# dvrp0/Monsoon

Hardware: AMD Instinct MI355X
Metric: env-steps/sec (whole node) at 65536 concurrent games; bit-exact vs CPU replay (higher is better)
Workload: dtype u8/i16 state, f64 draw+score

## Files before the change

monsoon_amd/csrc/msb_base.h:

```cpp
#pragma once
#include <stdint.h>

#if defined(__HIPCC__)
#include <hip/hip_runtime.h>
#define MSB_HD __device__
#define MSB_NOINLINE __attribute__((noinline))
#else
#define MSB_HD
#define MSB_NOINLINE __attribute__((noinline))
#endif
#define MSB_INL inline __attribute__((always_inline))

#define MSB_PROF_LDS 16
#if defined(MSB_PROF) && MSB_PROF && defined(__HIP_DEVICE_COMPILE__)
typedef __attribute__((address_space(3))) unsigned long long* msb_lds64;
typedef __attribute__((address_space(3))) unsigned* msb_lds32;
__device__ inline __attribute__((always_inline)) bool msb_prof_leader() {
  unsigned l = __builtin_amdgcn_mbcnt_hi(~0u, __builtin_amdgcn_mbcnt_lo(~0u, 0u));
  return (unsigned)__builtin_amdgcn_readfirstlane((int)l) == l;
}
struct ProfScope {
  unsigned long long t0;
  int id;
  __device__ inline __attribute__((always_inline)) explicit ProfScope(int i) : t0(__builtin_readcyclecounter()), id(i) {
    if (msb_prof_leader()) {
      unsigned long long pre = *(msb_lds64)(unsigned long)(MSB_PROF_LDS + 896);
      if (pre) {
        __hip_atomic_fetch_add((msb_lds64)(unsigned long)(MSB_PROF_LDS + 384 + 8 * id), t0 - pre, __ATOMIC_RELAXED, __HIP_MEMORY_SCOPE_WORKGROUP);
        *(msb_lds64)(unsigned long)(MSB_PROF_LDS + 896) = 0ull;
      }
    }
  }
  __device__ inline __attribute__((always_inline)) ~ProfScope() {
    unsigned long long now = __builtin_readcyclecounter();
    if (msb_prof_leader()) {
      __hip_atomic_fetch_add((msb_lds64)(unsigned long)(MSB_PROF_LDS + 8 * id), now - t0, __ATOMIC_RELAXED, __HIP_MEMORY_SCOPE_WORKGROUP);
      __hip_atomic_fetch_add((msb_lds32)(unsigned long)(MSB_PROF_LDS + 256 + 4 * id), 1u, __ATOMIC_RELAXED, __HIP_MEMORY_SCOPE_WORKGROUP);
      *(msb_lds64)(unsigned long)(MSB_PROF_LDS + 904) = now;
    }
  }
};
#define MSB_SCOPE(id) ProfScope msb_prof_scope_(id)
#define MSB_PRECALL()                                                                                   \
  do {                                                                                                  \
    if (msb_prof_leader()) *(msb_lds64)(unsigned long)(MSB_PROF_LDS + 896) = __builtin_readcyclecounter(); \
  } while (0)
#define MSB_POSTCALL(id)                                                                                \
  do {                                                                                                  \
    unsigned long long now_ = __builtin_readcyclecounter();                                             \
    if (msb_prof_leader()) {                                                                            \
      unsigned long long post_ = *(msb_lds64)(unsigned long)(MSB_PROF_LDS + 904);                       \
      if (post_ && now_ > post_)                                                                        \
        __hip_atomic_fetch_add((msb_lds64)(unsigned long)(MSB_PROF_LDS + 640 + 8 * (id)), now_ - post_, __ATOMIC_RELAXED, __HIP_MEMORY_SCOPE_WORKGROUP); \
      *(msb_lds64)(unsigned long)(MSB_PROF_LDS + 904) = 0ull;                                           \
    }                                                                                                   \
  } while (0)
#else
#define MSB_SCOPE(id)
#define MSB_PRECALL() do {} while (0)
#define MSB_POSTCALL(id) do {} while (0)
#endif
enum {
  PS_STEP, PS_PLAYER_PLAY, PS_NEW_ENTITY, PS_RUN_ABILITY, PS_ABILITY_ENTITY, PS_ABILITY_SPELL, PS_GET_TARGETS, PS_SHAPE_TILES,
  PS_SHAPE_TARGETS, PS_DEAL_DAMAGE, PS_DESTROY, PS_FRONT_LINE, PS_SET_PATH, PS_MOVE, PS_COMMAND, PS_FORCE_ATTACK, PS_DRAW,
  PS_FLIP, PS_NEXT_TURN, PS_LEGAL, PS_SHUFFLE, PS_SORTED_HEAD, PS_SPAWN, PS_RESPAWN, PS_TELEPORT, PS_PUSH_PULL, PS_EMPTY_FRONT,
  PS_BEGIN_STEP, PS_OBS_RAISES, PS_FEATURES, PS_COUNT
};


namespace msb {

enum : int { KIND_UNIT = 0, KIND_STRUCT = 1, KIND_SPELL = 2 };
enum : int { TR_NONE = -1, TR_ON_PLAY = 0, TR_ON_DEATH = 1, TR_BEFORE_ATTACKING = 2, TR_AFTER_ATTACKING = 3,
             TR_AFTER_SURVIVING = 4, TR_BEFORE_MOVING = 5, TR_TURN_START = 6, TR_TURN_END = 7 };
enum : int { ST_FROZEN = 0, ST_POISONED = 1, ST_CONFUSED = 2, ST_DISABLED = 3, ST_VITALIZED = 4 };
enum : int { PH_TURN_START = 0, PH_PLAY = 1, PH_TURN_END = 2 };
enum : int { UT_CONSTRUCT = 0, UT_FLAKE, UT_KNIGHT, UT_PIRATE, UT_RAVEN, UT_RODENT, UT_SATYR, UT_TOAD, UT_UNDEAD,
             UT_VIKING, UT_HERO, UT_DRAGON, UT_ELDER, UT_FELINE, UT_ANCIENT, UT_PRIMAL };
enum : int { TK_UNIT = 0, TK_STRUCTURE = 1, TK_ANY = 2 };
enum : int { TS_FRIENDLY = 0, TS_ENEMY = 1, TS_ANY = 2 };

enum : int {
  FAULT_NONE = 0,
  FAULT_PY_EXCEPTION = 1,
  FAULT_INT_CARD = 2,
  FAULT_CAPACITY = 16,
  FAULT_TRIG_STACK = 17,
  FAULT_DEPTH = 18,
  FAULT_RNG_OVERRUN = 19,
  FAULT_UNSUPPORTED = 20,
  FAULT_STATUS_SAT = 21,
  FAULT_CAP_REM = 22,
  FAULT_CAP_DECK = 23,
  FAULT_CAP_HAND = 24,
  FAULT_CAP_PATH = 25,
  FAULT_CAP_INST = 26,
  FAULT_BOT_BOUND = 27,
  FAULT_OPP_BOUND = 28,
  FAULT_WORK_STACK = 29,
};

struct TargetSpec {
  int8_t has, kind, side;
  uint16_t types, xtypes;
  int16_t limit;
  int8_t non_hero;
  uint8_t status, xstatus;
  int8_t base;
};
struct CardInfo {
  int8_t kind, faction;
  uint8_t cost, strength, movement;
  int8_t trigger, ff, has_ability;
  uint16_t types;
  int8_t first_type;
  int32_t int_id;
  TargetSpec tgt;
};

// ... 42 lines not shown
```

monsoon_amd/csrc/rules.h:

```cpp
#pragma once
#include "mt19937.h"
#include "pyset.h"
#include "state.h"

#if defined(MSB_FAULT_TRACE) && !defined(__HIPCC__)
#include <execinfo.h>
#include <stdio.h>
static inline void msb_fault_trace(int code) {
  void* bt[24];
  int n = backtrace(bt, 24);
  fprintf(stderr, "set_fault(%d)\n", code);
  backtrace_symbols_fd(bt, n, 2);
}
#endif

#if defined(MSB_COUNT_FRAMES) && !defined(__HIPCC__)
#define MSB_COUNT_EVENT(i_) msb_frame_count[i_]++
#define MSB_COUNT_MAX(i_, v_) (msb_frame_count[i_] = (v_) > msb_frame_count[i_] ? (v_) : msb_frame_count[i_])
static long long msb_frame_count[64];
#else
#define MSB_COUNT_EVENT(i_)
#define MSB_COUNT_MAX(i_, v_)
#endif

// ... 296 lines not shown
    for (int i = j; i + 1 < n; i++) m.st8(pl(o, P_DECK + i), m.ld8(pl(o, P_DECK + i + 1)));
#else
    for (int i = j; i + 1 < n; i++) {
      m.st32(pl(o, P_DECK + 4 * i), m.ld32(pl(o, P_DECK + 4 * (i + 1))));
      m.st8(pl(o, P_AGE + i), m.ld8(pl(o, P_AGE + i + 1)));
    }
    m.st8(pl(o, P_AGE + n - 1), 0);
#endif
    m.st8(pl(o, P_DECK_N), n - 1);
  }
  MSB_HD MSB_INL void hand_remove_at(int o, int j) {
    int n = pl_hand_n(o);
#if defined(MSB_EXT) && MSB_EXT
    for (int i = j; i + 1 < n; i++) m.st8(pl(o, P_HAND + i), m.ld8(pl(o, P_HAND + i + 1)));
#else
    for (int i = j; i + 1 < n; i++) m.st32(pl(o, P_HAND + 4 * i), m.ld32(pl(o, P_HAND + 4 * (i + 1))));
#endif
    m.st8(pl(o, P_HAND_N), n - 1);
  }
  MSB_HD MSB_INL void hand_push_from_deck(int o, int idx) {
    int hn = pl_hand_n(o);
    if (hn >= HAND_CAP) {
      set_fault(FAULT_CAP_HAND);
      return;
    }
#if defined(MSB_EXT) && MSB_EXT
    m.st8(pl(o, P_HAND + hn), deck_id(o, idx));
#else
    m.st32(pl(o, P_HAND + 4 * hn), m.ld32(pl(o, P_DECK + 4 * idx)));
#endif
    m.st8(pl(o, P_HAND_N), hn + 1);
  }
  MSB_HD MSB_INL uint32_t hand_handle(int o, int i) const {
#if defined(MSB_EXT) && MSB_EXT
    return (uint32_t)hand_id(o, i);
#else
    return m.ld32(pl(o, P_HAND + 4 * i));
#endif
  }
  MSB_HD MSB_INL void deck_push_handle(int o, uint32_t h) {
    int n = pl_deck_n(o);
    if (n >= DECK_CAP) {
      set_fault(FAULT_CAP_DECK);
      return;
    }
#if defined(MSB_EXT) && MSB_EXT
    m.st8(pl(o, P_DECK + n), (int)h);
#else
    m.st32(pl(o, P_DECK + 4 * n), h);
    m.st8(pl(o, P_AGE + n), 0);
#endif
    m.st8(pl(o, P_DECK_N), n + 1);
  }
  MSB_HD MSB_NOINLINE void push_new_instance(int o, bool to_hand, int card, int cost, int fl, int x) {
    int n = to_hand ? pl_hand_n(o) : pl_deck_n(o);
    if (n >= (to_hand ? HAND_CAP : DECK_CAP)) {
      set_fault(to_hand ? FAULT_CAP_HAND : FAULT_CAP_DECK);
      return;
    }
    int rec, wrec = -1;
#if defined(MSB_EXT) && MSB_EXT
    int id = inst_alloc(o);
    if (fault()) return;
    m.st8(pl(o, (to_hand ? P_HAND : P_DECK) + n), id);
    rec = pl(o, P_INST + 4 * id);
    wrec = pl(o, P_AGE + id);
    m.st8(pl(o, P_IPOS + id), IPOS_UNKNOWN);
#else
    rec = pl(o, (to_hand ? P_HAND : P_DECK) + 4 * n);
    if (!to_hand) wrec = pl(o, P_AGE + n);
#endif
    m.st8(rec, card);
    m.st8(rec + 1, cost);
    m.st8(rec + 2, fl);
    m.st8(rec + 3, x);
    if (wrec >= 0) m.st8(wrec, 0);
    m.st8(pl(o, to_hand ? P_HAND_N : P_DECK_N), n + 1);
  }

  MSB_HD MSB_INL int board_at(int tile) const { return m.ld8(OFF_BOARD + tile); }
  MSB_HD MSB_INL void board_put(int tile, int slot) { m.st8(OFF_BOARD + tile, slot); }

  MSB_HD MSB_INL static int ent(int e) { return OFF_ENT + ENT_SIZE * e; }
  static_assert(OFF_ENT % 16 == 0 && ENT_SIZE == 16 && OFF_PL % 16 == 0 && PL_SIZE % 16 == 0, "granule-aligned blocks");
  MSB_HD MSB_INL static int eg(int e) { return OFF_ENT / 16 + e; }
  MSB_HD MSB_INL static int pg(int order) { return OFF_PL / 16 + order * (PL_SIZE / 16); }
  MSB_HD MSB_INL int e_card(int e) const { return m.ld8g(eg(e), EO_CARD); }
  MSB_HD MSB_INL int e_flags(int e) const { return m.ld8g(eg(e), EO_FLAGS); }
  MSB_HD MSB_INL int e_owner(int e) const { return m.ld8g(eg(e), EO_FLAGS) & EF_OWNER; }
  MSB_HD MSB_INL bool e_ff(int e) const { return (m.ld8g(eg(e), EO_FLAGS) & EF_FF) != 0; }
  MSB_HD MSB_INL void e_set_flag(int e, int bit, bool on) {
    int f = m.ld8g(eg(e), EO_FLAGS);
    m.st8g(eg(e), EO_FLAGS, on ? (f | bit) : (f & ~bit));
  }
  MSB_HD MSB_INL P e_pos(int e) const { return tile_p(m.ld8g(eg(e), EO_POS)); }
  MSB_HD MSB_INL void e_set_pos(int e, P p) { m.st8g(eg(e), EO_POS, p_tile(p)); }
  MSB_HD MSB_INL int e_mov(int e) const { return m.ld8g(eg(e), EO_MOV); }
  MSB_HD MSB_INL int e_str(int e) const { return m.ld16g(eg(e), EO_STR); }
  MSB_HD MSB_INL void e_set_str(int e, int v) { m.st16g(eg(e), EO_STR, v); }
  MSB_HD MSB_INL int e_dmg(int e) const { return m.ld16g(eg(e), EO_DMG); }
  MSB_HD MSB_INL void e_set_dmg(int e, int v) { m.st16g(eg(e), EO_DMG, v); }
  MSB_HD MSB_INL int e_st(int e, int s) const { return m.ld8g(eg(e), EO_ST + s); }
  MSB_HD MSB_INL void e_st_add(int e, int s) {
    int c = m.ld8g(eg(e), EO_ST + s);
    if (c >= 255) {
      set_fault(FAULT_STATUS_SAT);
// ... 1057 lines not shown
      if (e_card_trigger(e) == TR_ON_DEATH) {
        push_trigger(e, src);
        if (fault()) return;
        if (!m.ld8(H_RESOLVING)) {
          wk_push(k, mk_hdr(F_DESTROY_TAIL, 0, 0, 0));
          call_pop_trigger(k);
          return;
        }
      }
      recalc_front_after_destroy();
    } else {
      e_set_dmg(e, e_str(e));
      board_set(e_pos(e), -1);
      recalc_front_after_destroy();
    }
  }
  MSB_HD MSB_INL bool need_unit(int e) {
    if (e < 0 || e >= AT_PLAYER || !e_is_unit(e)) {
      set_fault(FAULT_PY_EXCEPTION);
      return false;
    }
    return true;
  }
  MSB_HD MSB_INL void freeze(int e) {
    if (need_unit(e)) e_st_add(e, ST_FROZEN);
  }
  MSB_HD MSB_INL void poison(int e) {
    if (!need_unit(e)) return;
    if (e_st(e, ST_VITALIZED) > 0) e_st_remove(e, ST_VITALIZED);
    e_st_add(e, ST_POISONED);
  }
  MSB_HD MSB_INL void vitalize(int e) {
    if (!need_unit(e)) return;
    if (e_st(e, ST_POISONED) > 0) e_st_remove(e, ST_POISONED);
    e_st_add(e, ST_VITALIZED);
  }
  MSB_HD MSB_INL void confuse(int e) {
    if (need_unit(e)) e_st_add(e, ST_CONFUSED);
  }
  MSB_HD MSB_INL void deconfuse(int e) {
    if (need_unit(e)) e_st_remove(e, ST_CONFUSED);
  }
  MSB_HD MSB_INL void disable(int e) {
    if (need_unit(e) && e_has_ability(e)) e_st_add(e, ST_DISABLED);
  }

  MSB_HD MSB_INL void set_path(int e, bool on_play) {
    const int sv = ctx_enter(e);
    set_path_impl(e, on_play);
    ctx_leave(sv);
  }
  MSB_HD MSB_A_SETPATH void set_path_impl(int e, bool on_play) {
    MSB_SCOPE(PS_SET_PATH);
    P position = e_pos(e);
    int confused_cached = e_st(e, ST_CONFUSED);
    int owner = e_owner(e);
    bool is_local = owner == local();
    int steps = on_play ? e_mov(e) : 1;
    uint32_t packed = 0;
    int n = 0;
    unsigned long long dests = 0;
    int nd = 0;
    for (int k = 0; k < steps; k++) {
      P dest{position.x, position.y + (is_local ? -1 : 1)};
      int nxt = at(dest);
      if (confused_cached > 0) {
        int dx;
        if (position.x == 0)
          dx = 1;
        else if (position.x == 3)
          dx = -1;
        else
          dx = rng_randint(0, 2) ? 1 : -1;
        dest = P{position.x + dx, position.y};
        confused_cached--;
      } else if (on_play && !e_ff(e) && dest.y != (is_local ? -1 : 5) &&
                 (nxt == AT_NONE || (nxt < AT_PLAYER && e_owner(nxt) == owner))) {
        P lp{position.x - 1, position.y}, rp{position.x + 1, position.y};
        int left = position.x > 0 ? at(lp) : AT_NONE;
        int right = position.x < 3 ? at(rp) : AT_NONE;
        bool left_ok = left >= 0 && left < AT_PLAYER && e_owner(left) != owner;
        bool right_ok = right >= 0 && right < AT_PLAYER && e_owner(right) != owner;
        int lpk = p_pack(lp), rpk = p_pack(rp);
        bool lseen = false, rseen = false;
        for (int i = 0; i < nd; i++) {
          int dv = (int)((dests >> (8 * i)) & 0xff);
          if (dv == lpk) lseen = true;
          if (dv == rpk) rseen = true;
        }
        if (position.x <= 1) {
          if (right_ok && !rseen)
            dest = rp;
          else if (left_ok && !lseen)
            dest = lp;
        } else {
          if (left_ok && !lseen)
            dest = lp;
          else if (right_ok && !rseen)
            dest = rp;
        }
      }
      P enc = dest;
      if (enc.y < -1) enc.y = -1;
      if (enc.y > 5) enc.y = 5;
      if (nd < 8) dests |= (unsigned long long)p_pack(enc) << (8 * nd++);
      if (n < PATH_CAP) {
        packed |= (uint32_t)p_pack(enc) << (8 * n);
        n++;
      } else {
        set_fault(FAULT_CAP_PATH);
      }
      position = dest;
    }
    e_set_path(e, packed);
    m.st8g(eg(e), EO_PATHN, n);
  }

  enum : int { MV_ENTRY = 0, MV_POISONED, MV_BEFORE_MOVING, MV_STEP, MV_BASE_HIT, MV_FIGHT, MV_STRUCK, MV_STRUCK_BACK,
               MV_TARGET_DEAD, MV_SELF_DEAD, MV_AFTER_ATTACK, MV_DONE, MV_START };
  static constexpr int MV_PLAYED = 0x80;
  MSB_HD MSB_INL int move_enter(Wk& k, int e) {
    const int sv = ctx_enter(e);
    if (fault()) return -1;
    wk_push_ctx(k, sv);
    const int d = m.ld8(H_DEPTH);
    if (d >= MAX_DEPTH || !wk_reserve(k)) {
      MSB_COUNT_MAX(12, k.base + k.sp - k.seg);
      set_fault(d >= MAX_DEPTH ? FAULT_DEPTH : FAULT_WORK_STACK);
      return -1;
    }
    m.st8(H_DEPTH, d + 1);
    MSB_COUNT_MAX(13, d + 1);
    return d;
  }
  MSB_HD MSB_INL void call_move(Wk& k, int e, int played = 0) {
    const int d = move_enter(k, e);
    if (d < 0) return;
    k.sp += 3;
    wk_push(k, mk_hdr(F_MOVE, MV_ENTRY, e, d | played));
  }
  MSB_HD MSB_INL void call_move_later(Wk& k, int e, int played) {
    k.sp += 3;
    wk_push(k, mk_hdr(F_MOVE, MV_START, e, played));
  }
  MSB_HD MSB_INL void h_move(Wk& k, uint32_t hdr) {
    if (hdr_st(hdr) == MV_START) {
      const int e0 = hdr_a(hdr), played = hdr_b(hdr) & MV_PLAYED;
      k.sp -= 4;
      const int d0 = move_enter(k, e0);
      if (d0 < 0) return;
      k.sp += 4;
      hdr = mk_hdr(F_MOVE, MV_ENTRY, e0, d0 | played);
    }
    const int top = k.sp - 1;
    const int e = hdr_a(hdr), d = hdr_b(hdr) & 0x7f;
    const int played_tail = hdr_b(hdr) & MV_PLAYED;
    uint32_t path = 0, w2 = 0;
    int cached = 0;
    if (hdr_st(hdr) != MV_ENTRY) {
      path = m.sk_ld(top - 1);
      w2 = m.sk_ld(top - 2);
      cached = (int)(int16_t)(m.sk_ld(top - 3) & 0xffffu);
    }
    int i = (int)(w2 & 7), n = (int)((w2 >> 3) & 7), current_id = (int)((w2 >> 8) & 0xff), target = (int)((w2 >> 16) & 0xff);
    int flags = (int)(w2 >> 24);
    const int trig = e_trigger(e);
    int next = MV_DONE;
    P dest{0, 0};
// ... 314 lines not shown
    return !(acc / last <= u);
  }
  MSB_HD MSB_A_DRAW void draw(int o, int amount, int hint = 0) {
    MSB_SCOPE(PS_DRAW);
    for (int k = 0; k < amount; k++) {
      int n = pl_deck_n(o);
      if (n == 0) {
        set_fault(FAULT_PY_EXCEPTION);
        return;
      }
      int idx = 0;
      if (k == 0 && hint > 0) {
        (void)rng_random_sample();
        idx = hint - 1;
      } else {
        double sum = 0.0;
        for (int i = 0; i < n; i++) sum = sum + deck_w(o, i);
        double last = 0.0;
        for (int i = 0; i < n; i++) {
          double p = deck_w(o, i) / sum;
          last = (i == 0) ? p : last + p;
        }
        double u = rng_random_sample();
        double acc = 0.0;
        for (; idx < n; idx++) {
          double p = deck_w(o, idx) / sum;
          acc = (idx == 0) ? p : acc + p;
          if (draw_stops(acc, last, u)) break;
        }
#if defined(MSB_STUDY_DRAW)
        {
          double sum2 = 0.0, last2 = 0.0, acc2 = 0.0;
          for (int i = 0; i < n; i++) sum2 = sum2 + deck_w(o, i);
          asm volatile("" : "+v"(sum2));
          for (int i = 0; i < n; i++) {
            double p = deck_w(o, i) / sum2;
            last2 = (i == 0) ? p : last2 + p;
          }
          asm volatile("" : "+v"(last2));
          int idx2 = 0;
          for (; idx2 < n; idx2++) {
            double p = deck_w(o, idx2) / sum2;
            acc2 = (idx2 == 0) ? p : acc2 + p;
            if (draw_stops(acc2, last2, u)) break;
          }
          asm volatile("" : : "v"(idx2), "v"(acc2) : "memory");
        }
#endif
      }
      if (idx >= n) {
        set_fault(FAULT_PY_EXCEPTION);
        return;
      }
      set_deck_age(o, idx, 0);
      hand_push_from_deck(o, idx);
      if (fault()) return;
      int j = first_equal(o, false, idx);
      if (fault()) return;
      deck_remove_at(o, j);
    }
  }
  MSB_HD MSB_INL void fill_hand(int o) {
    int need = 4 - pl_hand_n(o);
    if (need > 0) draw(o, need);
  }
  MSB_HD MSB_INL void discard(int o, int hand_index) {
    reweight(o);
    if (fault()) return;
    uint32_t target = hand_handle(o, hand_index);
    int fl = hand_flags(o, hand_index);
    int j = first_equal(o, true, hand_index);
    if (fault()) return;
    hand_remove_at(o, j);
    if (!(fl & CF_SINGLE_USE)) deck_push_handle(o, target);
  }
  MSB_HD MSB_INL void add_history(int owner, int card) {
    int n = m.ld8(H_HIST_N);
    uint64_t h = m.ld64(H_HIST);
    const uint64_t entry = (uint64_t)(owner & 0xff) | ((uint64_t)(card & 0xff) << 8);
    if (n < 4) {
      h = (h & ~(0xffffull << (16 * n))) | (entry << (16 * n));
      m.st8(H_HIST_N, n + 1);
    } else {
      h = (h >> 16) | (entry << 48);
    }
    m.st64(H_HIST, h);
  }
  MSB_HD MSB_INL void call_player_play(Wk& k, int o, int index, P position, bool has_pos) {
    MSB_SCOPE(PS_PLAYER_PLAY);
    int card = hand_card(o, index), fl = hand_flags(o, index);
    int strength = inst_strength(card, fl, hand_x(o, index));
    add_history(o, card);
    discard(o, index);
    if (fault()) return;
    const CardInfo& ci = g_cards[card];
    if (ci.kind == KIND_UNIT) {
      int e = new_entity(card, o, strength, ci.movement, (fl & CF_FF) != 0);
      if (fault()) return;
      if (!has_pos) {
        set_fault(FAULT_PY_EXCEPTION);
        return;
      }
      call_unit_play(k, e, position);
    } else if (ci.kind == KIND_STRUCT) {
      int e = new_entity(card, o, strength, 0, false);
      if (fault()) return;
      if (fl & CF_SINGLE_USE) e_set_flag(e, EF_SINGLE_USE, true);
      if (!has_pos) {
        set_fault(FAULT_PY_EXCEPTION);
        return;
      }
      call_structure_play(k, e, position);
    } else {
      call_spell_play(k, card, o, position, has_pos);
    }
  }
  MSB_HD MSB_INL void call_spell_play(Wk& k, int card, int o, P position, bool has_pos) {
    const CardInfo& ci = g_cards[card];
    bool go = true;
    if (ci.tgt.has) {
      Tgt t = mk_tgt(ci.tgt);
      go = has_pos && target_has(cp(), t, position);
      if (!has_pos && targets_any(cp(), t)) {
        set_fault(FAULT_PY_EXCEPTION);
        return;
      }
    }
    if (go) call_run_ability(k, -1, card | (o << 8), has_pos ? p_pack(position) : PK_NONE, true);
  }
  MSB_HD MSB_INL void cycle(int o, int hand_index) {
#if MSB_COOP_DRAW && !(defined(MSB_EXT) && MSB_EXT)
    const int appended = !(hand_flags(o, hand_index) & CF_SINGLE_USE);
    discard(o, hand_index);
    if (fault()) return;
    draw(o, 1, (int)((M::draw_hint() >> (appended ? 0 : 8)) & 0xff));
#else
    discard(o, hand_index);
    if (fault()) return;
    draw(o, 1);
#endif
  }

  MSB_HD MSB_A_TURN void flip() {
    set_pl_front(0, 4 - pl_front(0));
    set_pl_front(1, 4 - pl_front(1));
    const uint32_t r0 = board_row(0), r1 = board_row(1), r2 = board_row(2), r3 = board_row(3), r4 = board_row(4);
    for (int y = 0; y < 5; y++) {
      uint32_t v = y == 0 ? r4 : y == 1 ? r3 : y == 2 ? r2 : y == 3 ? r1 : r0;
      v = (v >> 24) | ((v >> 8) & 0xff00u) | ((v << 8) & 0xff0000u) | (v << 24);
      m.st32(OFF_BOARD + 4 * y, v);
      for (int x = 0; x < 4; x++) {
        uint32_t s = (v >> (8 * x)) & 0xff;
        if (s != (uint32_t)SLOT_NONE) {
          m.st8g(eg((int)s), EO_POS, y * 4 + x);
          if (REM_LISTS) m.st8(E_HOME + (int)s, 0);
        }
      }
    }
  }
  MSB_HD MSB_INL void call_next_turn(Wk& k) {
    m.st8(H_PHASE, PH_TURN_END);
    int ender = cp();
    fill_hand(ender);
    if (fault()) return;
    calculate_front_line(local());
    calculate_front_line(remote());
    m.st16(pl(ender, P_MAXMANA), pl_maxmana(ender) + 1);
    set_pl_mana(0, pl_maxmana(0));
    set_pl_mana(1, pl_maxmana(1));
    m.st8(H_PHASE, PH_TURN_START);
    int ncp = (ender == local()) ? remote() : local();
    m.st8(H_CP, ncp);
    m.st8(pl(ncp, P_FLAGS), m.ld8(pl(ncp, P_FLAGS)) | 3);
    PList hs;
    hs.clear();
    PList snap = get_targets(ncp, mk_tgt(TK_STRUCTURE, TS_FRIENDLY), PK_NONE);
    int ns = snap.n();
    for (int i = 0; i < ns; i++) hs.set8(i, at(snap.at(i)));
    wk_push_list(k, hs);
    wk_push(k, mk_hdr(F_TURN, 0, 0, ns));
  }
  MSB_HD MSB_INL void h_turn(Wk& k, const uint32_t hdr) {
    const int top = k.sp - 1;
    int i = hdr_a(hdr), ns = hdr_b(hdr);
    PList hs = wk_list(top - 1, 0);
    if (hdr_st(hdr) == 0) {
      while (i < ns) {
// ... 57 lines not shown
        }
        if (place_row0) {
          MSB_SETBIT(155);
          any_play = true;
        }
      } else if (!ci.tgt.has) {
        MSB_SETBIT(64 + 21 * c);
        any_play = true;
      } else {
        PList l = get_targets(cp(), mk_tgt(ci.tgt), PK_NONE);
        int ln = l.n();
        for (int i = 0; i < ln; i++) {
          P p = l.at(i);
          MSB_SETBIT(p_valid(p) ? 65 + 21 * c + (4 - p.y) * 4 + p.x : 155);
          any_play = true;
        }
      }
    }
    if (m.ld8(pl(lo, P_FLAGS)) & 1)
      for (int c = 0; c < hn; c++) MSB_SETBIT(148 + c);
    if (!any_play) MSB_SETBIT(155);
#undef MSB_SETBIT
    return msb_u64x4{m0, m1, m2, 0ull};
  }
  MSB_HD MSB_INL void legal_mask(uint64_t mask[3]) {
    msb_u64x4 r = legal_mask_v();
    mask[0] = r[0];
    mask[1] = r[1];
    mask[2] = r[2];
  }

#if defined(MSB_STUDY_REPEAT)
  MSB_HD MSB_INL int step(int action, int cut = 0) { return step_impl(action, cut); }
  MSB_HD MSB_A_STEP int step_impl(int action, int cut) {
#define MSB_STUDY_CUT(n_) if (cut == (n_)) return 0;
#define MSB_STUDY_LIMIT (cut >= 3 ? cut - 2 : 1 << 30)
#else
  MSB_HD MSB_INL int step(int action) { return step_impl(action); }
  MSB_HD MSB_A_STEP int step_impl(int action) {
#define MSB_STUDY_CUT(n_)
#endif
    MSB_SCOPE(PS_STEP);
    Wk k{0, 0, 0, 0};
    begin_step();
    if (fault()) return 0;
    MSB_STUDY_CUT(1)
    int lo = local();
    if (action < 148) {
      bool place = action < 64;
      int ci = place ? action >> 4 : (action - 64) / 21;
      int idx = place ? action & 15 : (action - 64) % 21;
      if (idx < 20) {
        P pos{idx & 3, 4 - (idx >> 2)};
        bool has_pos = place || g_cards[hand_card(lo, ci)].tgt.has != 0;
        set_pl_mana(lo, pl_mana(lo) - hand_cost(lo, ci));
        call_player_play(k, lo, ci, pos, has_pos);
      }
    } else if (action < 152) {
      cycle(lo, action - 148);
      m.st8(pl(lo, P_FLAGS), m.ld8(pl(lo, P_FLAGS)) & ~1);
    } else if (action < 155) {
      int ci = action - 151;
#if defined(MSB_EXT) && MSB_EXT
      int a = hand_id(lo, ci), b = hand_id(lo, 0);
      m.st8(pl(lo, P_HAND + ci), b);
      m.st8(pl(lo, P_HAND), a);
#else
      uint32_t a = m.ld32(pl(lo, P_HAND + 4 * ci)), b = m.ld32(pl(lo, P_HAND));
      m.st32(pl(lo, P_HAND + 4 * ci), b);
      m.st32(pl(lo, P_HAND), a);
#endif
      m.st8(pl(lo, P_FLAGS), m.ld8(pl(lo, P_FLAGS)) & ~2);
    } else if (action == 155) {
      k.result = (pl_base(remote()) <= 0 ? 1 : 0) | (have_winner() ? 2 : 0);
      m.st8(H_TOPLAY, lo ^ 1);
      flip();
      k.sp = next_turn_out(k.sp);
    }
    MSB_STUDY_CUT(2)
#if defined(MSB_STUDY_REPEAT)
    run(k, MSB_STUDY_LIMIT);
#else
    run(k);
#endif
    if (fault()) return action == 155 ? k.result : 0;
    if (action != 155) k.result = (pl_base(remote()) <= 0 ? 1 : 0) | (have_winner() ? 2 : 0);
    if (m.ld8(H_RNGOVER)) set_fault(FAULT_RNG_OVERRUN);
    return k.result;
  }

  MSB_HD MSB_INL void h_ctx_leave(Wk& k, const uint32_t hdr) {
    ctx_leave(hdr_a(hdr));
    k.sp--;
  }
  MSB_HD MSB_INL void h_destroy_tail(Wk& k, const uint32_t) {
    recalc_front_after_destroy();
    k.sp--;
  }
  MSB_HD MSB_INL void h_cmd_tail(Wk& k, const uint32_t hdr) {
    e_set_flag(hdr_a(hdr), EF_FF, hdr_b(hdr) != 0);
    k.sp--;
  }
  MSB_HD MSB_INL void wk_dispatch(Wk& k, int fn, const uint32_t hdr) {
    switch (fn) {
      case F_MOVE: {
        MSB_SCOPE(PS_MOVE);
        h_move(k, hdr);
      } break;
      case F_RUNAB: {
// ... 232 lines not shown
```

monsoon_amd/csrc/state.h:

```cpp
#pragma once
#include "msb_base.h"
#include "lds_layout.h"

namespace msb {

#if defined(MSB_CAP_ENT)
constexpr int NUM_ENT = MSB_CAP_ENT;
#elif defined(MSB_EXT) && MSB_EXT == 2
constexpr int NUM_ENT = 254;
#elif defined(MSB_EXT) && MSB_EXT
constexpr int NUM_ENT = 64;
#else
constexpr int NUM_ENT = 24;
#endif
constexpr int HAND_CAP = 5;
constexpr int DECK_SIZE = 12;
#if defined(MSB_EXT) && MSB_EXT
#if MSB_EXT == 2
constexpr int DECK_CAP = 48;
#else
constexpr int DECK_CAP = 28;
#endif
#if defined(MSB_CAP_REM)
constexpr int REM_LISTS = MSB_CAP_REM, WORLD_CAP = MSB_CAP_WORLD;
// ... 46 lines not shown
constexpr int H_HIST = 8;
constexpr int H_USED = 16;
constexpr int H_RNGPOS = 20;
constexpr int H_OBSFAULT = 22;
constexpr int GF_OBSFAULT = 1, GF_ALIAS = 2;
constexpr int H_RNGOVER = 23;
constexpr int OFF_BOARD = 24;
constexpr int OFF_TRIG = 44;
constexpr int H_RNGCUR = 64;
constexpr int H_RNGNXT = 72;
constexpr int OFF_PL = 80;

constexpr int P_BASE = 0;
constexpr int P_MANA = 2;
constexpr int P_MAXMANA = 4;
constexpr int P_FRONT = 6;
constexpr int P_FLAGS = 7;
constexpr int P_FACTION = 8;
constexpr int P_HAND_N = 9;
constexpr int P_DECK_N = 10;
#if defined(MSB_EXT) && MSB_EXT
constexpr int INST_CAP = DECK_CAP + 8;
constexpr int P_HAND = 12;
constexpr int P_DECK = P_HAND + HAND_CAP;
constexpr int P_INST = (P_DECK + DECK_CAP + 3) & ~3;
constexpr int P_AGE = P_INST + 4 * INST_CAP;
constexpr int P_IPOS = P_AGE + INST_CAP;
constexpr int IPOS_UNKNOWN = 0xFF;
constexpr int PL_SIZE = (P_IPOS + INST_CAP + 15) & ~15;
#else
constexpr int P_HAND = 12;
constexpr int P_DECK = P_HAND + 4 * HAND_CAP;
constexpr int P_AGE = P_DECK + 4 * DECK_CAP;
constexpr int PL_SIZE = (P_AGE + DECK_CAP + 15) & ~15;
#endif
static_assert((OFF_PL % 16) == 0 && (PL_SIZE % 16) == 0 && (P_AGE % 4) == 0, "granule / word alignment");
constexpr int AGE_MAX = 255;
constexpr int WT_LDS_N = 32;
#if defined(MSB_PROF) && MSB_PROF
constexpr int WT_LDS = 928;
#else
constexpr int WT_LDS = 16;
#endif
constexpr int WK_OVF_LDS = WT_LDS + 8 * WT_LDS_N;
constexpr int DRAW_HINT_LDS = WK_OVF_LDS + 8;
#ifndef MSB_COOP_DRAW
#define MSB_COOP_DRAW 1
#endif
#ifndef MSB_COOP_LEGAL
#define MSB_COOP_LEGAL 1
#endif
#ifndef MSB_TARGET_SCAN
#define MSB_TARGET_SCAN 1
#endif
constexpr int LDS_RECORDS = WK_OVF_LDS + 16;
constexpr int SK_CAP = 640;
constexpr int SK_MARGIN = 32;
constexpr int SK_NEED = 12;
constexpr int CF_SINGLE_USE = 1, CF_FF = 2, CF_STR = 4, CF_ALIAS = 8;
constexpr int CF_XBASE = 16, CF_SPELL = 32;

constexpr int OFF_ENT = (OFF_PL + 2 * PL_SIZE + 15) & ~15;
constexpr int ENT_SIZE = 16;
constexpr int EO_CARD = 0;
constexpr int EO_FLAGS = 1;
constexpr int EO_POS = 2;
constexpr int EO_MOV = 3;
constexpr int EO_ST = 4;
constexpr int EO_MOVEID = 9;
constexpr int EO_STR = 10;
constexpr int EO_DMG = 12;
constexpr int EO_PATHN = 14;
constexpr int EO_KIND = 15;
constexpr int EK_UNIT = 1, EK_ABILITY = 2;
constexpr int E_PATH = OFF_ENT + ENT_SIZE * NUM_ENT;
constexpr int E_REM = E_PATH + 4 * NUM_ENT;
constexpr int E_HOME = E_REM + (REM_LISTS ? NUM_ENT : 0);
constexpr int OFF_REM = (E_HOME + (REM_LISTS ? NUM_ENT : 0) + 3) & ~3;
constexpr int OFF_WORLD = (OFF_REM + REM_LISTS * REM_LIST_BYTES + 3) & ~3;
constexpr int USED_WORDS = (NUM_ENT + 31) / 32;
constexpr bool TRIG_WIDE = NUM_ENT > 128;
constexpr int TRIG_SLOT = TRIG_WIDE ? 0xff : 0x7f;
constexpr int OFF_X = OFF_WORLD + WORLD_CAP * WORLD_BYTES;
constexpr int X_CTX = OFF_X, X_RNGBLK = OFF_X + 2, X_SEED = OFF_X + 4, X_USED_HI = OFF_X + 8;
constexpr int X_TRIGSRC = X_USED_HI + 4 * (USED_WORDS - 1);
constexpr int X_BYTES = REM_LISTS ? (X_TRIGSRC - OFF_X) + (TRIG_WIDE ? 4 : 0) : 0;
constexpr int STATE_BYTES = (OFF_X + X_BYTES + 15) & ~15;
static_assert(NUM_ENT <= 254 && (!TRIG_WIDE || REM_LISTS), "slot ids are bytes; 0xFE and 0xFF are markers");
constexpr int STATE_WORDS = STATE_BYTES / 4;
#ifndef MSB_LDS_COLUMNS
#define MSB_LDS_COLUMNS 1
#endif
#ifndef MSB_LDS_COLUMNS_LARGE
#define MSB_LDS_COLUMNS_LARGE 0
#endif
#if !(defined(MSB_EXT) && MSB_EXT)
constexpr bool PLAY_LDS_COLUMNS = MSB_LDS_COLUMNS;
#elif MSB_EXT == 2
constexpr bool PLAY_LDS_COLUMNS = MSB_LDS_COLUMNS && MSB_LDS_COLUMNS_LARGE;
#else
constexpr bool PLAY_LDS_COLUMNS = false;
#endif
static_assert(!PLAY_LDS_COLUMNS || lds_layout::stride_conflict_free(STATE_BYTES), "columns need a record of +-16 bytes (mod 128)");
constexpr int EF_OWNER = 1, EF_FF = 2, EF_RESOLVING_PLAY = 4, EF_SINGLE_USE = 8;
typedef uint32_t msb_u32x4 __attribute__((vector_size(16)));

// ... 277 lines not shown
```

Before: 2.043 billion.

## Rewrite hand/deck list ops and path setup with wide 128-bit granule accesses

Adds wide variants of discard and draw-take that load each player's hand, deck and age granules as 128-bit vectors and update them in registers with branchless byte masks, replacing many byte/word LDS accesses and separate helper calls. A second path-setup variant reads the entity header word once and decodes fields from it. Both are enabled by default via new macros, and the old paths are kept. This trades more ALU work and register pressure for fewer LDS transactions, at the risk of subtle bit-exactness differences in fault ordering.

```diff
diff --git a/monsoon_amd/csrc/msb_base.h b/monsoon_amd/csrc/msb_base.h
--- a/monsoon_amd/csrc/msb_base.h
+++ b/monsoon_amd/csrc/msb_base.h
@@ -64,7 +64,7 @@
   PS_STEP, PS_PLAYER_PLAY, PS_NEW_ENTITY, PS_RUN_ABILITY, PS_ABILITY_ENTITY, PS_ABILITY_SPELL, PS_GET_TARGETS, PS_SHAPE_TILES,
   PS_SHAPE_TARGETS, PS_DEAL_DAMAGE, PS_DESTROY, PS_FRONT_LINE, PS_SET_PATH, PS_MOVE, PS_COMMAND, PS_FORCE_ATTACK, PS_DRAW,
   PS_FLIP, PS_NEXT_TURN, PS_LEGAL, PS_SHUFFLE, PS_SORTED_HEAD, PS_SPAWN, PS_RESPAWN, PS_TELEPORT, PS_PUSH_PULL, PS_EMPTY_FRONT,
-  PS_BEGIN_STEP, PS_OBS_RAISES, PS_FEATURES, PS_COUNT
+  PS_BEGIN_STEP, PS_OBS_RAISES, PS_FEATURES, PS_DISCARD, PS_COUNT
 };
 
 
diff --git a/monsoon_amd/csrc/rules.h b/monsoon_amd/csrc/rules.h
--- a/monsoon_amd/csrc/rules.h
+++ b/monsoon_amd/csrc/rules.h
@@ -372,6 +372,129 @@
 #endif
     m.st8(pl(o, P_DECK_N), n + 1);
   }
+#if !(defined(MSB_EXT) && MSB_EXT)
+  static_assert(P_FACTION == 8 && P_HAND_N == 9 && P_DECK_N == 10 && P_HAND == 12 && P_DECK == 32 && P_AGE == 80 && PL_SIZE == 96 &&
+                    HAND_CAP == 5 && DECK_CAP == 12,
+                "the six granules of a player block");
+  MSB_HD MSB_INL static uint32_t bits_to_bytes(uint32_t bits) { return (((bits & 0xfu) * 0x00204081u) & 0x01010101u) * 0xffu; }
+  MSB_HD MSB_INL static uint32_t pl_counts(uint32_t hdr, int hand_n, int deck_n) {
+    return (hdr & 0xff0000ffu) | ((uint32_t)(hand_n & 0xff) << 8) | ((uint32_t)(deck_n & 0xff) << 16);
+  }
+  MSB_HD MSB_INL static int first_equal_fault(uint32_t first, int positioned) {
+    const int pi = (int)(first >> 16) & (CF_ALIAS | CF_STR);
+    if (!pi && !positioned) return 0;
+    return (pi && positioned) ? FAULT_UNSUPPORTED : FAULT_PY_EXCEPTION;
+  }
+  MSB_HD MSB_INL bool discard_wide(int o, int idx, uint32_t target) {
+    const int g = pg(o);
+    msb_u32x4 g0 = m.ld128g(g), g1 = m.ld128g(g + 1);
+    const msb_u32x4 ga = m.ld128g(g + 5);
+    const int faulted = fault();
+    const int hn = (int)(g0[2] >> 8) & 0xff, dn = (int)(g0[2] >> 16) & 0xff;
+    uint32_t a[3] = {ga[0], ga[1], ga[2]};
+    bool stop = false;
+    for (int w = 0; w < 3; w++) {
+      const int k = dn - 4 * w;
+      const uint32_t t = ~a[w];
+      stop = stop || (k > 0 && ((t - 0x01010101u) & ~t & 0x80808080u) != 0);
+      const uint32_t one = k >= 4 ? 0x01010101u : (k > 0 ? (0x01010101u >> (8 * (4 - k))) : 0u);
+      a[w] = stop ? a[w] : a[w] + one;
+    }
+    if (stop || faulted) {
+      m.st128g(g + 5, msb_u32x4{a[0], a[1], a[2], ga[3]});
+      if (stop) set_fault(FAULT_CAP_DECK);
+      return false;
+    }
+    const uint32_t h[5] = {g0[3], g1[0], g1[1], g1[2], g1[3]};
+    const uint32_t card = target & 0xffu;
+    uint32_t eq = 0;
+    for (int i = 0; i < 5; i++) eq |= (uint32_t)((h[i] & 0xffu) == card) << i;
+    eq &= (1u << idx) - 1u;
+    int j = idx;
+    if (eq != 0 && card_eq_by_id((int)card)) {
+      j = __builtin_ctz(eq);
+      const uint32_t first = j == 0 ? h[0] : (j == 1 ? h[1] : (j == 2 ? h[2] : h[3]));
+      const int code = first_equal_fault(first, (int)(target >> 16) & (CF_ALIAS | CF_STR));
+      if (code) {
+        m.st128g(g + 5, msb_u32x4{a[0], a[1], a[2], ga[3]});
+        set_fault(code);
+        return false;
+      }
+    }
+    uint32_t nh[5];
+    for (int i = 0; i < 4; i++) nh[i] = (i >= j && i + 1 < hn) ? h[i + 1] : h[i];
+    nh[4] = h[4];
+    int dn2 = dn;
+    bool full = false;
+    if (!((target >> 16) & CF_SINGLE_USE)) {
+      full = dn >= DECK_CAP;
+      if (!full) {
+        m.st32(pl(o, P_DECK + 4 * dn), target);
+        const uint32_t keep = ~(0xffu << (8 * (dn & 3)));
+        for (int w = 0; w < 3; w++) a[w] = (dn >> 2) == w ? (a[w] & keep) : a[w];
+        dn2 = dn + 1;
+      }
+    }
+    g0[2] = pl_counts(g0[2], hn - 1, dn2);
+    g0[3] = nh[0];
+    m.st128g(g, g0);
+    m.st128g(g + 1, msb_u32x4{nh[1], nh[2], nh[3], nh[4]});
+    m.st128g(g + 5, msb_u32x4{a[0], a[1], a[2], ga[3]});
+    if (full) set_fault(FAULT_CAP_DECK);
+    return !full;
+  }
+  MSB_HD MSB_INL bool draw_take_wide(int o, int idx) {
+    const int g = pg(o);
+    const uint32_t hdr = m.ld32g(g, P_FACTION);
+    const uint32_t choice = m.ld32(pl(o, P_DECK + 4 * idx));
+    const msb_u32x4 d0 = m.ld128g(g + 2), d1 = m.ld128g(g + 3), d2 = m.ld128g(g + 4), ga = m.ld128g(g + 5);
+    const int faulted = fault();
+    const int hn = (int)(hdr >> 8) & 0xff, n = (int)(hdr >> 16) & 0xff;
+    uint32_t a[3] = {ga[0], ga[1], ga[2]};
+    {
+      const uint32_t keep = ~(0xffu << (8 * (idx & 3)));
+      for (int w = 0; w < 3; w++) a[w] = (idx >> 2) == w ? (a[w] & keep) : a[w];
+    }
+    if (hn >= HAND_CAP) {
+      m.st128g(g + 5, msb_u32x4{a[0], a[1], a[2], ga[3]});
+      set_fault(FAULT_CAP_HAND);
+      return false;
+    }
+    m.st32(pl(o, P_HAND + 4 * hn), choice);
+    const uint32_t d[12] = {d0[0], d0[1], d0[2], d0[3], d1[0], d1[1], d1[2], d1[3], d2[0], d2[1], d2[2], d2[3]};
+    const uint32_t card = choice & 0xffu;
+    uint32_t eq = 0;
+    for (int i = 0; i < 12; i++) eq |= (uint32_t)((d[i] & 0xffu) == card) << i;
+    eq &= (1u << idx) - 1u;
+    int j = idx, code = 0;
+    if (!faulted && eq != 0 && card_eq_by_id((int)card)) {
+      j = __builtin_ctz(eq);
+      code = first_equal_fault(m.ld32(pl(o, P_DECK + 4 * j)), (int)(choice >> 16) & (CF_ALIAS | CF_STR));
+    }
+    if (faulted || code) {
+      m.st32g(g, P_FACTION, pl_counts(hdr, hn + 1, n));
+      m.st128g(g + 5, msb_u32x4{a[0], a[1], a[2], ga[3]});
+      if (code) set_fault(code);
+      return false;
+    }
+    const uint32_t take = ((1u << (n - 1)) - 1u) & ~((1u << j) - 1u), zero = 1u << (n - 1);
+    uint32_t nd[12];
+    for (int i = 0; i < 11; i++) nd[i] = ((take >> i) & 1u) ? d[i + 1] : d[i];
+    nd[11] = d[11];
+    uint32_t na[3];
+    for (int w = 0; w < 3; w++) {
+      const uint32_t down = (a[w] >> 8) | (w < 2 ? a[w < 2 ? w + 1 : 2] << 24 : 0u);
+      const uint32_t tb = bits_to_bytes(take >> (4 * w)), zb = bits_to_bytes(zero >> (4 * w));
+      na[w] = (a[w] & ~(tb | zb)) | (down & tb);
+    }
+    m.st128g(g + 2, msb_u32x4{nd[0], nd[1], nd[2], nd[3]});
+    m.st128g(g + 3, msb_u32x4{nd[4], nd[5], nd[6], nd[7]});
+    m.st128g(g + 4, msb_u32x4{nd[8], nd[9], nd[10], nd[11]});
+    m.st128g(g + 5, msb_u32x4{na[0], na[1], na[2], ga[3]});
+    m.st32g(g, P_FACTION, pl_counts(hdr, hn + 1, n - 1));
+    return true;
+  }
+#endif
   MSB_HD MSB_NOINLINE void push_new_instance(int o, bool to_hand, int card, int cost, int fl, int x) {
     int n = to_hand ? pl_hand_n(o) : pl_deck_n(o);
     if (n >= (to_hand ? HAND_CAP : DECK_CAP)) {
@@ -1535,6 +1658,73 @@
   }
   MSB_HD MSB_A_SETPATH void set_path_impl(int e, bool on_play) {
     MSB_SCOPE(PS_SET_PATH);
+#if MSB_WIDE_PATH
+    static_assert(EO_CARD == 0 && EO_FLAGS == 1 && EO_POS == 2 && EO_MOV == 3, "word 0 of an entity");
+    const uint32_t ge = m.ld32g(eg(e), 0);
+    P position = tile_p((int)(ge >> 16) & 0xff);
+    int confused_cached = e_st(e, ST_CONFUSED);
+    const int owner = (int)(ge >> 8) & EF_OWNER;
+    const bool ff = ((ge >> 8) & EF_FF) != 0;
+    const bool is_local = owner == local();
+    const int steps = on_play ? (int)(ge >> 24) : 1;
+    uint32_t packed = 0;
+    int n = 0, nd = 0;
+    uint32_t seen = 0;
+    for (int k = 0; k < steps; k++) {
+      P dest{position.x, position.y + (is_local ? -1 : 1)};
+      if (confused_cached > 0) {
+        int dx;
+        if (position.x == 0)
+          dx = 1;
+        else if (position.x == 3)
+          dx = -1;
+        else
+          dx = rng_randint(0, 2) ? 1 : -1;
+        dest = P{position.x + dx, position.y};
+        confused_cached--;
+      } else if (on_play && !ff && dest.y != (is_local ? -1 : 5)) {
+        const uint32_t row = (position.y >= 0 && position.y <= 4) ? board_row(position.y) : 0xffffffffu;
+        const uint32_t ahead = (dest.y >= 0 && dest.y <= 4) ? board_row(dest.y) : 0xffffffffu;
+        const int x = position.x;
+        const int nxt = (int)(ahead >> (8 * x)) & 0xff;
+        const int left = x > 0 ? (int)(row >> (8 * (x > 0 ? x - 1 : 0))) & 0xff : SLOT_NONE;
+        const int right = x < 3 ? (int)(row >> (8 * (x < 3 ? x + 1 : 3))) & 0xff : SLOT_NONE;
+        const int fn = m.ld8g(eg(nxt == SLOT_NONE ? e : nxt), EO_FLAGS), fl = m.ld8g(eg(left == SLOT_NONE ? e : left), EO_FLAGS),
+                  fr = m.ld8g(eg(right == SLOT_NONE ? e : right), EO_FLAGS);
+        if (nxt == SLOT_NONE || (fn & EF_OWNER) == owner) {
+          const bool left_ok = left != SLOT_NONE && (fl & EF_OWNER) != owner && !((seen >> ((position.y * 4 + x - 1) & 31)) & 1u);
+          const bool right_ok = right != SLOT_NONE && (fr & EF_OWNER) != owner && !((seen >> ((position.y * 4 + x + 1) & 31)) & 1u);
+          if (x <= 1) {
+            if (right_ok)
+              dest = P{x + 1, position.y};
+            else if (left_ok)
+              dest = P{x - 1, position.y};
+          } else {
+            if (left_ok)
+              dest = P{x - 1, position.y};
+            else if (right_ok)
+              dest = P{x + 1, position.y};
+          }
+        }
+      }
+      P enc = dest;
+      if (enc.y < -1) enc.y = -1;
+      if (enc.y > 5) enc.y = 5;
+      if (nd < 8) {
+        if (p_valid(enc)) seen |= 1u << p_tile(enc);
+        nd++;
+      }
+      if (n < PATH_CAP) {
+        packed |= (uint32_t)p_pack(enc) << (8 * n);
+        n++;
+      } else {
+        set_fault(FAULT_CAP_PATH);
+      }
+      position = dest;
+    }
+    e_set_path(e, packed);
+    m.st8g(eg(e), EO_PATHN, n);
+#else
     P position = e_pos(e);
     int confused_cached = e_st(e, ST_CONFUSED);
     int owner = e_owner(e);
@@ -1597,6 +1787,7 @@
     }
     e_set_path(e, packed);
     m.st8g(eg(e), EO_PATHN, n);
+#endif
   }
 
   enum : int { MV_ENTRY = 0, MV_POISONED, MV_BEFORE_MOVING, MV_STEP, MV_BASE_HIT, MV_FIGHT, MV_STRUCK, MV_STRUCK_BACK,
@@ -2017,19 +2208,31 @@
         set_fault(FAULT_PY_EXCEPTION);
         return;
       }
+#if MSB_WIDE_LISTS && !(defined(MSB_EXT) && MSB_EXT)
+      if (!draw_take_wide(o, idx)) return;
+#else
       set_deck_age(o, idx, 0);
       hand_push_from_deck(o, idx);
       if (fault()) return;
       int j = first_equal(o, false, idx);
       if (fault()) return;
       deck_remove_at(o, j);
+#endif
     }
   }
   MSB_HD MSB_INL void fill_hand(int o) {
     int need = 4 - pl_hand_n(o);
     if (need > 0) draw(o, need);
   }
+#if MSB_WIDE_LISTS && !(defined(MSB_EXT) && MSB_EXT)
+  MSB_HD MSB_INL bool discard(int o, int hand_index, uint32_t entry) {
+    MSB_SCOPE(PS_DISCARD);
+    return discard_wide(o, hand_index, entry);
+  }
+  MSB_HD MSB_INL void discard(int o, int hand_index) { discard(o, hand_index, hand_handle(o, hand_index)); }
+#else
   MSB_HD MSB_INL void discard(int o, int hand_index) {
+    MSB_SCOPE(PS_DISCARD);
     reweight(o);
     if (fault()) return;
     uint32_t target = hand_handle(o, hand_index);
@@ -2039,6 +2242,7 @@
     hand_remove_at(o, j);
     if (!(fl & CF_SINGLE_USE)) deck_push_handle(o, target);
   }
+#endif
   MSB_HD MSB_INL void add_history(int owner, int card) {
     int n = m.ld8(H_HIST_N);
     uint64_t h = m.ld64(H_HIST);
@@ -2051,6 +2255,17 @@
     }
     m.st64(H_HIST, h);
   }
+#if MSB_WIDE_LISTS && !(defined(MSB_EXT) && MSB_EXT)
+  MSB_HD MSB_INL void call_player_play(Wk& k, int o, int index, P position, bool has_pos) {
+    call_player_play(k, o, index, hand_handle(o, index), position, has_pos);
+  }
+  MSB_HD MSB_INL void call_player_play(Wk& k, int o, int index, uint32_t entry, P position, bool has_pos) {
+    MSB_SCOPE(PS_PLAYER_PLAY);
+    int card = (int)(entry & 0xffu), fl = (int)(entry >> 16) & 0xff;
+    int strength = inst_strength(card, fl, (int)(entry >> 24));
+    add_history(o, card);
+    if (!discard(o, index, entry)) return;
+#else
   MSB_HD MSB_INL void call_player_play(Wk& k, int o, int index, P position, bool has_pos) {
     MSB_SCOPE(PS_PLAYER_PLAY);
     int card = hand_card(o, index), fl = hand_flags(o, index);
@@ -2058,6 +2273,7 @@
     add_history(o, card);
     discard(o, index);
     if (fault()) return;
+#endif
     const CardInfo& ci = g_cards[card];
     if (ci.kind == KIND_UNIT) {
       int e = new_entity(card, o, strength, ci.movement, (fl & CF_FF) != 0);
@@ -2095,9 +2311,15 @@
   }
   MSB_HD MSB_INL void cycle(int o, int hand_index) {
 #if MSB_COOP_DRAW && !(defined(MSB_EXT) && MSB_EXT)
+#if MSB_WIDE_LISTS
+    const uint32_t entry = hand_handle(o, hand_index);
+    const int appended = !((entry >> 16) & CF_SINGLE_USE);
+    if (!discard(o, hand_index, entry)) return;
+#else
     const int appended = !(hand_flags(o, hand_index) & CF_SINGLE_USE);
     discard(o, hand_index);
     if (fault()) return;
+#endif
     draw(o, 1, (int)((M::draw_hint() >> (appended ? 0 : 8)) & 0xff));
 #else
     discard(o, hand_index);
@@ -2261,9 +2483,16 @@
       int idx = place ? action & 15 : (action - 64) % 21;
       if (idx < 20) {
         P pos{idx & 3, 4 - (idx >> 2)};
+#if MSB_WIDE_LISTS && !(defined(MSB_EXT) && MSB_EXT)
+        const uint32_t entry = hand_handle(lo, ci);
+        bool has_pos = place || g_cards[entry & 0xffu].tgt.has != 0;
+        set_pl_mana(lo, pl_mana(lo) - (int)((entry >> 8) & 0xffu));
+        call_player_play(k, lo, ci, entry, pos, has_pos);
+#else
         bool has_pos = place || g_cards[hand_card(lo, ci)].tgt.has != 0;
         set_pl_mana(lo, pl_mana(lo) - hand_cost(lo, ci));
         call_player_play(k, lo, ci, pos, has_pos);
+#endif
       }
     } else if (action < 152) {
       cycle(lo, action - 148);
diff --git a/monsoon_amd/csrc/state.h b/monsoon_amd/csrc/state.h
--- a/monsoon_amd/csrc/state.h
+++ b/monsoon_amd/csrc/state.h
@@ -122,6 +122,12 @@
 #endif
 #ifndef MSB_TARGET_SCAN
 #define MSB_TARGET_SCAN 1
+#endif
+#ifndef MSB_WIDE_LISTS
+#define MSB_WIDE_LISTS 1
+#endif
+#ifndef MSB_WIDE_PATH
+#define MSB_WIDE_PATH 1
 #endif
 constexpr int LDS_RECORDS = WK_OVF_LDS + 16;
 constexpr int SK_CAP = 640;
```

After: 2.110 billion, median of 6. 1.03x the previous value.
